# ElusAegis/metal-msm-gpu-acceleration

Hardware: AMD Instinct MI355X
Metric: BN254 G1 MSM/s at log_size=20 (5 instances) (higher is better)
Workload: dtype u32x8 (256-bit Montgomery integer)

## Files before the change

### include/msm_amd.h

```cpp
#ifndef MSM_AMD_H
#define MSM_AMD_H

#include <stddef.h>
#include <stdint.h>

#ifdef __cplusplus
extern "C" {
#endif

typedef struct msm_amd_ctx msm_amd_ctx;

enum {
  MSM_AMD_OK = 0,
  MSM_AMD_DEVICE_NOT_FOUND = 1,
  MSM_AMD_LIBRARY_ERROR = 2,
  MSM_AMD_FUNCTION_ERROR = 3,
  MSM_AMD_PIPELINE_ERROR = 4,
  MSM_AMD_INPUT_ERROR = 5,
  MSM_AMD_FILE_OPEN_ERROR = 6,
  MSM_AMD_DESERIALIZATION_ERROR = 7,
  MSM_AMD_INVALID_DATA = 8
};

enum {
// ... 235 lines not shown
  MSM_AMD_RAW_FE_SQR_WIDE = 33,
  MSM_AMD_RAW_FE_MUL2_WIDE = 34
};
int msm_amd_test_op_raw(msm_amd_ctx* ctx, int op, const uint32_t* a, const uint32_t* b, uint32_t* out, size_t count);
int msm_amd_test_op_raw_host(int op, const uint32_t* a, const uint32_t* b, uint32_t* out, size_t count);

int msm_amd_test_hold(msm_amd_ctx* ctx, uint32_t max_ms, void** handle);
int msm_amd_test_release(msm_amd_ctx* ctx, void* handle);

enum {
  MSM_AMD_TP_C = 0, MSM_AMD_TP_W, MSM_AMD_TP_W_DIGITS, MSM_AMD_TP_N, MSM_AMD_TP_N_SCALARS, MSM_AMD_TP_LB, MSM_AMD_TP_NB,
  MSM_AMD_TP_CH, MSM_AMD_TP_HB, MSM_AMD_TP_MB, MSM_AMD_TP_FB, MSM_AMD_TP_Q, MSM_AMD_TP_TILED, MSM_AMD_TP_BALLOT,
  MSM_AMD_TP_WIDE_DIGITS, MSM_AMD_TP_LONE,
  MSM_AMD_TP_TOTAL_ITEMS, MSM_AMD_TP_MULTI_COUNT, MSM_AMD_TP_DEFERRED,
  MSM_AMD_TP_RED_GROUP, MSM_AMD_TP_RB_THREADS, MSM_AMD_TP_INSTANCES, MSM_AMD_TP_WORKSPACE, MSM_AMD_TP_FRONT_THREADS,
  MSM_AMD_TEST_PLAN_WORDS
};
int msm_amd_test_last_plan(msm_amd_ctx* ctx, uint32_t j, uint32_t* out, size_t count);
enum {
  MSM_AMD_STAGE_DIGITS = 0,
  MSM_AMD_STAGE_SORTED = 1,
  MSM_AMD_STAGE_BUCKET_SIZE = 2,
  MSM_AMD_STAGE_BUCKET_START = 3,
  MSM_AMD_STAGE_ITEM_START = 4,
  MSM_AMD_STAGE_WIN_ITEMS = 5,
  MSM_AMD_STAGE_ORDER = 6,
  MSM_AMD_STAGE_MULTI_LIST = 7,
  MSM_AMD_STAGE_BUCKETS = 8,
  MSM_AMD_STAGE_PARTIAL = 9
};
// ... 63 lines not shown
```

### metal-msm-gpu-acceleration_amd/__init__.py

```python
from __future__ import annotations

import ctypes
import os
from ctypes import POINTER, c_char_p, c_float, c_int, c_size_t, c_uint32, c_uint64, c_void_p

_HERE = os.path.dirname(os.path.abspath(__file__))
LIB_PATH = os.environ.get("MSM_AMD_LIB") or os.path.join(_HERE, "libmsm_amd.so")

(OK, DEVICE_NOT_FOUND, LIBRARY_ERROR, FUNCTION_ERROR, PIPELINE_ERROR, INPUT_ERROR, FILE_OPEN_ERROR,
 DESERIALIZATION_ERROR, INVALID_DATA) = range(9)
SCALAR_MONT_LE, SCALAR_CANON_LE, SCALAR_CANON_BE32 = 0, 1, 2
POINT_H2C_AFFINE, POINT_ARK_PROJECTIVE, POINT_ARK_AFFINE, POINT_JAC_BE32, POINT_PREPARED, POINT_TABLES = 0, 1, 2, 3, 4, 5
POINT_BYTES = {POINT_H2C_AFFINE: 64, POINT_ARK_PROJECTIVE: 96, POINT_ARK_AFFINE: 72, POINT_JAC_BE32: 96}
(OP_UINT_ADD, OP_UINT_SUB, OP_UINT_PROD, OP_UINT_SHL, OP_UINT_SHR, OP_FP_ADD, OP_FP_SUB, OP_FP_MUL, OP_FP_NEG,
 OP_FP_POW, OP_EC_ADD, OP_EC_MUL, OP_EC_MADD, OP_EC_DBL, OP_FP29_MUL, OP_FP29_SQR, OP_FP29_SUB_K4E30,
 OP_FP29_SUB_K8E30, OP_FP29_SUB_K8E31, OP_FP29_SUB_K16E30, OP_FP29_SUB_K16E31, OP_FP29_ROUNDTRIP, OP_EC29_MADD,
 OP_EC29_ADD, OP_EC29_MADD_CHAIN, OP_EC29_ADD_CHAIN, OP_EC29_MMADD, OP_H64_FP_MUL, OP_H64_FP_ADD, OP_H64_FP_SUB,
 OP_H64_EC_ADD, OP_H64_EC_DBL, OP_FP29_MUL_KARATSUBA, OP_FP29_LOCKSTEP_PAIR, OP_FP29_LOCKSTEP_MIX,
 OP_FP29_LOCKSTEP_TRIPLE, OP_FP29_MUL2_KARATSUBA, OP_H64_FP_INV, OP_H64_FP_INV_FERMAT) = range(39)
(RAW_FE_MUL, RAW_FE_SQR, RAW_FE_MUL2, RAW_FE_SUB_K4E30, RAW_FE_SUB_K8E30, RAW_FE_SUB_K8E31, RAW_FE_SUB_K16E30,
 RAW_FE_SUB_K16E31, RAW_FE_NORM, RAW_FE_NEG, RAW_FE_NEG_WIDE, RAW_FE_CANONICAL, RAW_FE_TO_EXT, RAW_FE_PACK_UNPACK,
 RAW_FE_ZERO, RAW_PT_MADD, RAW_PT_MMADD, RAW_PT_ADD_NZ, RAW_PT_ADD, RAW_PT_DOUBLE) = range(20)
RAW_FE_MUL_WIDE, RAW_FE_SQR_WIDE, RAW_FE_MUL2_WIDE = range(32, 35)
RAW_IN_WORDS, RAW_OUT_WORDS = 36, 40
# ... 32 lines not shown
    "msm_amd_set_bases_cache_verify",
    "msm_amd_scalar_bytes", "msm_amd_point_bytes", "msm_amd_shard_owner",
    "msm_amd_shard_count", "msm_amd_ctx_device", "msm_amd_pin_thread_to_device", "msm_amd_gather_init",
    "msm_amd_gather_size", "msm_amd_gather_all", "msm_amd_gather_last_error", "msm_amd_gather_destroy",
    "msm_amd_host_msm", "msm_amd_tuned_split", "msm_amd_host_threads", "msm_amd_generate_instance_host", "msm_amd_test_op_ifma",
    "msm_amd_test_last_plan", "msm_amd_test_stage_copy", "msm_amd_test_fill_workspaces",
    "msm_amd_g2_point_bytes", "msm_amd_msm_g2", "msm_amd_msm_g2_device", "msm_amd_host_msm_g2",
    "msm_amd_test_g2_progression", "msm_amd_test_op_g2", "msm_amd_test_op_g2_host",
    "msm_amd_g2_bases_upload", "msm_amd_g2_bases_prepare_device", "msm_amd_msm_g2_prepared",
    "msm_amd_g2_tables_build", "msm_amd_g2_tables_build_device", "msm_amd_g2_tables_info", "msm_amd_g2_tables_free",
    "msm_amd_msm_g2_tables", "msm_amd_test_g2_tables_read", "msm_amd_test_g2_table_host",
]

TEST_PLAN_FIELDS = ("c", "W", "W_digits", "n", "n_scalars", "lb", "nb", "CH", "hb", "mb", "fb", "Q", "tiled", "ballot",
                    "wide_digits", "lone", "total_items", "multi_count", "deferred", "red_group", "rb_threads",
                    "instances", "workspace", "front_threads")
(STAGE_DIGITS, STAGE_SORTED, STAGE_BUCKET_SIZE, STAGE_BUCKET_START, STAGE_ITEM_START, STAGE_WIN_ITEMS, STAGE_ORDER,
 STAGE_MULTI_LIST, STAGE_BUCKETS, STAGE_PARTIAL) = range(10)


AFTER_SORT_FN = ctypes.CFUNCTYPE(None, c_void_p)


class Timings(ctypes.Structure):
    _fields_ = [("convert_ms", c_float), ("digits_ms", c_float), ("sort_ms", c_float), ("accumulate_ms", c_float),
                ("reduce_ms", c_float), ("final_ms", c_float), ("total_gpu_ms", c_float), ("n", c_uint32),
                ("window_size", c_uint32), ("num_windows", c_uint32), ("reserved", c_uint32),
                ("accumulate_kernel_ms", c_float), ("reserved2", c_float * 3)]


class MsmError(RuntimeError):
# ... 741 lines not shown
```

### metal-msm-gpu-acceleration_amd/csrc/k_sort.hip

```cpp
#include <algorithm>

#include "device_common.hip.h"
#include "launch.h"

namespace msm_amd {

constexpr int kSortThreads = 1024;

template <typename D, int C = 0>
__global__ void __launch_bounds__(256)
digits_kernel(const u256* __restrict__ scalars, uint32_t n, uint32_t c_arg, uint32_t W_arg, int scalars_mont,
              D* __restrict__ digits) {
  constexpr uint32_t kSignShift = 8 * sizeof(D) - 1;
  const uint32_t c = C > 0 ? (uint32_t)C : c_arg;
  const uint32_t W = C > 0 ? (uint32_t)(254 / (C > 0 ? C : 1) + 1) : W_arg;
  __builtin_amdgcn_s_setprio(kFrontPriority);
  const uint32_t t = blockIdx.x * blockDim.x + threadIdx.x;
  if (t >= n) return;
  u256 k = load_u256(&scalars[t]);
  if (scalars_mont) {
    k = Fr::from_mont(k);
  } else {
#pragma unroll 1
    for (int i = 0; i < 5; ++i) k = Fr::reduce_once(k);
  }
  const uint32_t half = 1u << (c - 1);
  uint32_t carry = 0;
#pragma unroll
  for (uint32_t w = 0; w < W; ++w) {
    const uint32_t start = w * c;
    uint32_t v = (start < 256 ? u256_extract_bits(k, start, c) : 0u) + carry;
    uint32_t neg = 0;
    carry = 0;
    if (v > half) {
      v = (1u << c) - v;
      neg = 1;
      carry = 1;
    }
    digits[(size_t)w * n + t] = (D)(v | (neg << kSignShift));
  }
}

constexpr uint32_t kFineCap = 28672;

template <typename D>
__global__ void __launch_bounds__(kSortThreads)
coarse_hist_kernel(const D* __restrict__ digits, uint32_t n, uint32_t fb, uint32_t nhi, uint32_t chunk,
                   uint32_t* __restrict__ coarse_cnt ) {
  constexpr uint32_t kMagMask = (1u << (8 * sizeof(D) - 1)) - 1u;
  __builtin_amdgcn_s_setprio(kFrontPriority);
  extern __shared__ uint32_t lds_u32[];
  const uint32_t q = blockIdx.x, Q = gridDim.x, w = blockIdx.y;
  for (uint32_t i = threadIdx.x; i < nhi; i += blockDim.x) lds_u32[i] = 0;
  __syncthreads();
// ... 48 lines not shown
    hi &= ~((uint32_t)(bal >> 32) ^ (uint32_t)s);
  }
  const uint32_t rank = __builtin_amdgcn_mbcnt_hi(hi, __builtin_amdgcn_mbcnt_lo(lo, 0u));
  const uint32_t count = __popc(lo) + __popc(hi);
  const uint32_t leader = lo ? (uint32_t)__builtin_ctz(lo) : 32u + (uint32_t)__builtin_ctz(hi | 0x80000000u);
  uint32_t base = 0;
  if (valid && rank == 0) base = atomicAdd(&cursors[key], count);
  base = (uint32_t)__builtin_amdgcn_ds_bpermute((int)(leader << 2), (int)base);
  return base + rank;
}

template <typename D, bool BALLOT>
__global__ void __launch_bounds__(kSortThreads)
coarse_scatter_kernel(const D* __restrict__ digits, uint32_t n, uint32_t hb, uint32_t fb, uint32_t chunk,
                      const uint32_t* __restrict__ coarse_base , uint32_t* __restrict__ tmp_idx,
                      uint16_t* __restrict__ tmp_fine) {
  __builtin_amdgcn_s_setprio(kFrontPriority);
  extern __shared__ uint32_t lds_u32[];
  const uint32_t nhi = 1u << hb;
  const uint32_t q = blockIdx.x, Q = gridDim.x, w = blockIdx.y;
  const uint32_t* base = coarse_base + ((size_t)w * Q + q) * nhi;
  for (uint32_t i = threadIdx.x; i < nhi; i += blockDim.x) lds_u32[i] = base[i];
  __syncthreads();
  const uint32_t lo = q * chunk;
  const uint32_t hi_end = min(n, lo + chunk);
  constexpr uint32_t kSignShift = 8 * sizeof(D) - 1;
  constexpr uint32_t kMagMask = (1u << kSignShift) - 1u;
  const D* dw = digits + (size_t)w * n;
  uint32_t* ti = tmp_idx + (size_t)w * n;
  uint16_t* tf = tmp_fine + (size_t)w * n;
  const uint32_t fmask = (1u << fb) - 1u;
  if (BALLOT) {
    for (uint32_t t0 = lo; t0 < hi_end; t0 += blockDim.x) {
      const uint32_t t = t0 + threadIdx.x;
      const uint32_t v = t < hi_end ? (uint32_t)dw[t] : 0u;
      const uint32_t m = v & kMagMask;
      const uint32_t slot = m - 1;
      const uint32_t pos = wave_claim(m ? slot >> fb : 0u, hb, m != 0, lds_u32);
      if (m) {
        ti[pos] = t | ((v >> kSignShift) << 31);
        tf[pos] = (uint16_t)(slot & fmask);
      }
    }
    return;
  }
  for (uint32_t t = lo + threadIdx.x; t < hi_end; t += blockDim.x) {
    const uint32_t v = dw[t];
    const uint32_t m = v & kMagMask;
    if (m) {
      const uint32_t slot = m - 1;
      const uint32_t pos = atomicAdd(&lds_u32[slot >> fb], 1u);
      ti[pos] = t | ((v >> kSignShift) << 31);
      tf[pos] = (uint16_t)(slot & fmask);
    }
  }
}


__global__ void __launch_bounds__(kSortThreads)
mid_hist_kernel(const uint16_t* __restrict__ tmp_fine, uint32_t n, uint32_t nhi, uint32_t fb, uint32_t nmid,
                const uint32_t* __restrict__ region_start, uint32_t* __restrict__ mid_cnt ) {
  __builtin_amdgcn_s_setprio(kFrontPriority);
  extern __shared__ uint32_t lds_u32[];
  const uint32_t q = blockIdx.x, Q2 = gridDim.x, R = blockIdx.y, w = R / nhi, r = R % nhi;
  for (uint32_t i = threadIdx.x; i < nmid; i += blockDim.x) lds_u32[i] = 0;
  __syncthreads();
  const uint32_t rs = region_start[(size_t)w * (nhi + 1) + r], re = region_start[(size_t)w * (nhi + 1) + r + 1];
  const uint32_t chunk = (((re - rs) + Q2 - 1) / Q2 + 63u) & ~63u;
// ... 123 lines not shown
#pragma unroll
    for (uint32_t e = 0; e < kTilePerThread; ++e) {
      if (reg[e] != 0xFFFFFFFFu) {
        const uint32_t p = off[reg[e]] + rank[e];
        st_idx[p] = pay[e];
        st_fine[p] = (uint16_t)fin[e];
        st_reg[p] = (uint8_t)reg[e];
      }
    }
    __syncthreads();
    const uint32_t tile_total = scratch[32];
    for (uint32_t j = threadIdx.x; j < tile_total; j += blockDim.x) {
      const uint32_t r = st_reg[j];
      const uint32_t gp = gbase[r] + (j - off[r]);
      out_idx[gp] = st_idx[j];
      out_fine[gp] = st_fine[j];
    }
    __syncthreads();
  }
}

template <typename D>
__global__ void __launch_bounds__(kSortThreads)
coarse_scatter_tiled_kernel(const D* __restrict__ digits, uint32_t n, uint32_t hb, uint32_t fb, uint32_t chunk,
                            const uint32_t* __restrict__ coarse_base, uint32_t* __restrict__ tmp_idx,
                            uint16_t* __restrict__ tmp_fine) {
  __builtin_amdgcn_s_setprio(kFrontPriority);
  extern __shared__ uint32_t lds_u32[];
  constexpr uint32_t kSignShift = 8 * sizeof(D) - 1;
  constexpr uint32_t kMagMask = (1u << kSignShift) - 1u;
  const uint32_t nhi = 1u << hb;
  const uint32_t q = blockIdx.x, Q = gridDim.x, w = blockIdx.y;
  const uint32_t lo = q * chunk, hi = min(n, lo + chunk);
  const D* dw = digits + (size_t)w * n;
  const uint32_t fmask = (1u << fb) - 1u;
  auto load = [&](uint32_t t, uint32_t* pay, uint32_t* fin, uint32_t* reg) {
    const uint32_t v = dw[t];
    const uint32_t m = v & kMagMask;
    if (!m) return false;
    const uint32_t slot = m - 1;
    *pay = t | ((v >> kSignShift) << 31);
    *fin = slot & fmask;
    *reg = slot >> fb;
    return true;
  };
  tile_scatter(lo, hi, nhi, hb, load, coarse_base + ((size_t)w * Q + q) * nhi, tmp_idx + (size_t)w * n,
               tmp_fine + (size_t)w * n, lds_u32);
}

__global__ void __launch_bounds__(kSortThreads)
mid_scatter_tiled_kernel(const uint32_t* __restrict__ tmp_idx, const uint16_t* __restrict__ tmp_fine, uint32_t n,
                         uint32_t nhi, uint32_t fb, uint32_t mb, const uint32_t* __restrict__ region_start,
                         const uint32_t* __restrict__ mid_base, uint32_t* __restrict__ tmp_idx2,
                         uint16_t* __restrict__ tmp_fine2) {
  __builtin_amdgcn_s_setprio(kFrontPriority);
  extern __shared__ uint32_t lds_u32[];
  const uint32_t nmid = 1u << mb;
  const uint32_t q = blockIdx.x, Q2 = gridDim.x, R = blockIdx.y, w = R / nhi, r = R % nhi;
  const uint32_t rs = region_start[(size_t)w * (nhi + 1) + r], re = region_start[(size_t)w * (nhi + 1) + r + 1];
  const uint32_t chunk = (((re - rs) + Q2 - 1) / Q2 + 63u) & ~63u;
  const uint32_t lo = min(re, rs + q * chunk), hi = min(re, lo + chunk);
  const uint32_t* ti = tmp_idx + (size_t)w * n;
  const uint16_t* tf = tmp_fine + (size_t)w * n;
  const uint32_t fmask = (1u << fb) - 1u;
  auto load = [&](uint32_t t, uint32_t* pay, uint32_t* fin, uint32_t* reg) {
    const uint32_t f = tf[t];
    *pay = ti[t];
    *fin = f & fmask;
    *reg = f >> fb;
    return true;
  };
  tile_scatter(lo, hi, nmid, mb, load, mid_base + ((size_t)R * Q2 + q) * nmid, tmp_idx2 + (size_t)w * n,
               tmp_fine2 + (size_t)w * n, lds_u32);
}

template <bool BALLOT>
__global__ void __launch_bounds__(kSortThreads)
fine_sort_kernel(const uint32_t* __restrict__ tmp_idx, const uint16_t* __restrict__ tmp_fine, uint32_t n,
                 uint32_t lb, uint32_t fb, const uint32_t* __restrict__ region_start,
                 uint32_t* __restrict__ sorted, uint32_t* __restrict__ bucket_size) {
  __builtin_amdgcn_s_setprio(kFrontPriority);
  extern __shared__ uint32_t lds_u32[];
  const uint32_t nfine = 1u << fb;
  const uint32_t nhi = gridDim.x;
  const uint32_t hi = blockIdx.x, w = blockIdx.y;
  uint32_t* bins = lds_u32;
  uint32_t* scratch = lds_u32 + nfine;
  uint32_t* staging = lds_u32 + nfine + 32;
  const uint32_t rs = region_start[(size_t)w * (nhi + 1) + hi];
  const uint32_t re = region_start[(size_t)w * (nhi + 1) + hi + 1];
  const uint32_t size = re - rs;
  const uint32_t* ti = tmp_idx + (size_t)w * n + rs;
  const uint16_t* tf = tmp_fine + (size_t)w * n + rs;
  uint32_t* out = sorted + (size_t)w * n + rs;
  for (uint32_t i = threadIdx.x; i < nfine; i += blockDim.x) bins[i] = 0;
  __syncthreads();
#pragma unroll 1
  for (uint32_t i = threadIdx.x; i < size; i += blockDim.x) atomicAdd(&bins[tf[i]], 1u);
  __syncthreads();
  const uint32_t cnt = (threadIdx.x < nfine) ? bins[threadIdx.x] : 0u;
  uint32_t total;
  const uint32_t start = block_exclusive_scan(cnt, scratch, &total);
  if (threadIdx.x < nfine) {
    bins[threadIdx.x] = start;
    const uint32_t slot = (hi << fb) | threadIdx.x;
    if (slot < (1u << lb)) bucket_size[((size_t)w << lb) + slot] = cnt;
  }
  __syncthreads();
  if (size <= kFineCap) {
    if (BALLOT) {
#pragma unroll 1
      for (uint32_t i0 = 0; i0 < size; i0 += blockDim.x) {
        const uint32_t i = i0 + threadIdx.x;
        const bool valid = i < size;
        const uint32_t pos = wave_claim(valid ? (uint32_t)tf[i] : 0u, fb, valid, bins);
        if (valid) staging[pos] = ti[i];
      }
    } else {
#pragma unroll 1
      for (uint32_t i = threadIdx.x; i < size; i += blockDim.x) {
        const uint32_t pos = atomicAdd(&bins[tf[i]], 1u);
        staging[pos] = ti[i];
      }
    }
    __syncthreads();
  #pragma unroll 1
  for (uint32_t i = threadIdx.x; i < size; i += blockDim.x) out[i] = staging[i];
  } else {
  #pragma unroll 1
  for (uint32_t i = threadIdx.x; i < size; i += blockDim.x) {
      const uint32_t pos = atomicAdd(&bins[tf[i]], 1u);
      out[pos] = ti[i];
    }
  }
}

__device__ __forceinline__ uint32_t window_scan_lds(uint32_t* tot, uint32_t* scratch, uint32_t nb) {
  const uint32_t per = (nb + blockDim.x - 1) / blockDim.x;
  const uint32_t first = threadIdx.x * per;
  uint32_t local = 0;
#pragma unroll 1
  for (uint32_t j = 0; j < per; ++j) {
    const uint32_t d = first + j;
    if (d < nb) local += tot[d + (d >> 5)];
  }
  uint32_t total;
  uint32_t run = block_exclusive_scan(local, scratch, &total);
// ... 209 lines not shown
  const size_t tile = std::min<size_t>((size_t)1 << lb, kPlanTile);
  return (tile + (tile >> 5) + 33) * 4;
}

int sort_set_attributes(const char** failed) {
  const int max_lds = 160 * 1024;
  struct { const void* fn; const char* name; } ks[] = {
      {(const void*)plan_kernel, "plan_kernel"},
      {(const void*)coarse_scatter_kernel<uint16_t, false>, "coarse_scatter_kernel<u16>"},
      {(const void*)coarse_scatter_kernel<uint32_t, false>, "coarse_scatter_kernel<u32>"},
      {(const void*)coarse_scatter_kernel<uint16_t, true>, "coarse_scatter_kernel<u16, ballot>"},
      {(const void*)coarse_scatter_kernel<uint32_t, true>, "coarse_scatter_kernel<u32, ballot>"},
      {(const void*)coarse_scatter_tiled_kernel<uint16_t>, "coarse_scatter_tiled_kernel<u16>"},
      {(const void*)coarse_scatter_tiled_kernel<uint32_t>, "coarse_scatter_tiled_kernel<u32>"},
      {(const void*)mid_scatter_tiled_kernel, "mid_scatter_tiled_kernel"},
      {(const void*)fine_sort_kernel<false>, "fine_sort_kernel"},
      {(const void*)fine_sort_kernel<true>, "fine_sort_kernel<ballot>"}};
  for (auto& k : ks) {
    if (hipFuncSetAttribute(k.fn, hipFuncAttributeMaxDynamicSharedMemorySize, max_lds) != hipSuccess) {
      (void)hipGetLastError();
      *failed = k.name;
      return 1;
    }
  }
  return 0;
}

void launch_digits(hipStream_t st, const Plan& p, const u256* scalars, int scalars_mont, void* digits) {
  const dim3 grid((p.n_scalars + 255) / 256), block(256);
#define LAUNCH_DIGITS_C(D, CC)                                                                                      \
  hipLaunchKernelGGL((digits_kernel<D, CC>), grid, block, 0, st, scalars, p.n_scalars, p.c, p.W_digits, scalars_mont, \
                     (D*)digits)
  if (p.W_digits == 254 / p.c + 1) {
    if (p.wide_digits && p.c == 17) { LAUNCH_DIGITS_C(uint32_t, 17); return; }
    if (p.wide_digits && p.c == 16) { LAUNCH_DIGITS_C(uint32_t, 16); return; }
    if (!p.wide_digits && p.c == 15) { LAUNCH_DIGITS_C(uint16_t, 15); return; }
    if (!p.wide_digits && p.c == 13) { LAUNCH_DIGITS_C(uint16_t, 13); return; }
  }
#undef LAUNCH_DIGITS_C
  if (p.wide_digits)
    hipLaunchKernelGGL(digits_kernel<uint32_t>, grid, block, 0, st, scalars, p.n_scalars, p.c, p.W_digits, scalars_mont,
                       (uint32_t*)digits);
  else
    hipLaunchKernelGGL(digits_kernel<uint16_t>, grid, block, 0, st, scalars, p.n_scalars, p.c, p.W_digits, scalars_mont,
                       (uint16_t*)digits);
}

void launch_sort(hipStream_t st, const Plan& p, const SortBuffers& b) {
  const uint32_t nhi = 1u << p.hb, nmid = 1u << p.mb, nfine = 1u << p.fb;
  const uint32_t fb1 = p.mb + p.fb;
  if (p.wide_digits)
    hipLaunchKernelGGL(coarse_hist_kernel<uint32_t>, dim3(p.Q, p.W), dim3(p.front_threads), nhi * 4, st,
                       (const uint32_t*)b.digits, p.n, fb1, nhi, p.chunk, b.coarse_cnt);
  else
    hipLaunchKernelGGL(coarse_hist_kernel<uint16_t>, dim3(p.Q, p.W), dim3(p.front_threads), nhi * 4, st,
                       (const uint16_t*)b.digits, p.n, fb1, nhi, p.chunk, b.coarse_cnt);
  hipLaunchKernelGGL(coarse_prefix_kernel, dim3(p.W), dim3(1024), 0, st, b.coarse_cnt, p.Q, nhi, b.region_start);
  const bool bc = (p.ballot & 1u) != 0, bf = (p.ballot & 2u) != 0;
#define LAUNCH_COARSE_SCATTER(D, B)                                                                                 \
  hipLaunchKernelGGL((coarse_scatter_kernel<D, B>), dim3(p.Q, p.W), dim3(p.front_threads), nhi * 4, st,             \
                     (const D*)b.digits, p.n, p.hb, fb1, p.chunk, (const uint32_t*)b.coarse_cnt, b.tmp_idx, b.tmp_fine)
  const bool tiled = p.tiled && p.front_threads == kSortThreads && nhi <= kTileMaxRegions && nmid <= kTileMaxRegions;
  if (tiled) {
    if (p.wide_digits)
      hipLaunchKernelGGL(coarse_scatter_tiled_kernel<uint32_t>, dim3(p.Q, p.W), dim3(p.tile_threads), kTileLdsBytes, st,
                         (const uint32_t*)b.digits, p.n, p.hb, fb1, p.chunk, (const uint32_t*)b.coarse_cnt, b.tmp_idx,
                         b.tmp_fine);
    else
      hipLaunchKernelGGL(coarse_scatter_tiled_kernel<uint16_t>, dim3(p.Q, p.W), dim3(p.tile_threads), kTileLdsBytes, st,
                         (const uint16_t*)b.digits, p.n, p.hb, fb1, p.chunk, (const uint32_t*)b.coarse_cnt, b.tmp_idx,
                         b.tmp_fine);
  } else if (p.wide_digits) {
    if (bc) LAUNCH_COARSE_SCATTER(uint32_t, true); else LAUNCH_COARSE_SCATTER(uint32_t, false);
  } else {
    if (bc) LAUNCH_COARSE_SCATTER(uint16_t, true); else LAUNCH_COARSE_SCATTER(uint16_t, false);
  }
#undef LAUNCH_COARSE_SCATTER
  const uint32_t* fine_idx = b.tmp_idx;
  const uint16_t* fine_fine = b.tmp_fine;
  const uint32_t* fine_regions = b.region_start;
  uint32_t fine_nhi = nhi;
  if (p.mb) {
    hipLaunchKernelGGL(mid_hist_kernel, dim3(p.Q2, nhi * p.W), dim3(p.front_threads), nmid * 4, st,
                       (const uint16_t*)b.tmp_fine, p.n, nhi, p.fb, nmid, (const uint32_t*)b.region_start, b.mid_cnt);
    hipLaunchKernelGGL(mid_prefix_kernel, dim3(nhi * p.W), dim3(1024), 0, st, b.mid_cnt, p.Q2, nhi, nmid,
                       (const uint32_t*)b.region_start, b.region_start2);
// ... 2 lines not shown
                         (const uint32_t*)b.tmp_idx, (const uint16_t*)b.tmp_fine, p.n, nhi, p.fb, p.mb,
                         (const uint32_t*)b.region_start, (const uint32_t*)b.mid_cnt, b.tmp_idx2, b.tmp_fine2);
    else if (bc)
      hipLaunchKernelGGL(mid_scatter_kernel<true>, dim3(p.Q2, nhi * p.W), dim3(p.front_threads), nmid * 4, st,
                         (const uint32_t*)b.tmp_idx, (const uint16_t*)b.tmp_fine, p.n, nhi, p.fb, nmid,
                         (const uint32_t*)b.region_start, (const uint32_t*)b.mid_cnt, b.tmp_idx2, b.tmp_fine2);
    else
      hipLaunchKernelGGL(mid_scatter_kernel<false>, dim3(p.Q2, nhi * p.W), dim3(p.front_threads), nmid * 4, st,
                         (const uint32_t*)b.tmp_idx, (const uint16_t*)b.tmp_fine, p.n, nhi, p.fb, nmid,
                         (const uint32_t*)b.region_start, (const uint32_t*)b.mid_cnt, b.tmp_idx2, b.tmp_fine2);
    fine_idx = b.tmp_idx2;
    fine_fine = b.tmp_fine2;
    fine_regions = b.region_start2;
    fine_nhi = nhi * nmid;
  }
  if (bf)
    hipLaunchKernelGGL(fine_sort_kernel<true>, dim3(fine_nhi, p.W), dim3(std::max(p.front_threads, nfine)),
                       (kFineCap + nfine + 32) * 4, st, fine_idx, fine_fine, p.n, p.lb, p.fb, fine_regions, b.sorted,
                       b.bucket_size);
  else
    hipLaunchKernelGGL(fine_sort_kernel<false>, dim3(fine_nhi, p.W), dim3(std::max(p.front_threads, nfine)),
                       (kFineCap + nfine + 32) * 4, st, fine_idx, fine_fine, p.n, p.lb, p.fb, fine_regions, b.sorted,
                       b.bucket_size);
  const unsigned tiles = (unsigned)((p.nb + kPlanTile - 1) / kPlanTile);
  if (tiles > 1)
    hipLaunchKernelGGL(plan_tile_sums_kernel, dim3(tiles, p.W), dim3(p.front_threads), 0, st,
                       (const uint32_t*)b.bucket_size, p.lb, p.CH, b.tile_sums);
  hipLaunchKernelGGL(plan_kernel, dim3(tiles, p.W), dim3(p.front_threads), lds_plan_bytes(p.lb), st,
                     (const uint32_t*)b.bucket_size, p.lb, p.CH, (const uint2*)b.tile_sums, b.bucket_start,
                     b.item_start, b.win_items);
  const unsigned size_threads = p.front_threads;
  const unsigned gb = (unsigned)((p.total_buckets + size_threads * kSizeChunks - 1) / (size_threads * kSizeChunks));
  hipLaunchKernelGGL(size_hist_kernel, dim3(gb), dim3(size_threads), (p.CH + 1) * 4, st,
                     (const uint32_t*)b.bucket_size, (uint32_t)p.total_buckets, p.CH, b.size_bins);
  hipLaunchKernelGGL(size_scan_kernel, dim3(1), dim3(1024), 0, st, b.size_bins, (p.CH + 1) * gb, b.win_items, p.W,
                     b.counters);
  hipLaunchKernelGGL(size_scatter_kernel, dim3(gb), dim3(size_threads), (2 * (p.CH + 1) + 2) * 4, st,
                     (const uint32_t*)b.bucket_size, (uint32_t)p.total_buckets, p.CH, (const uint32_t*)b.size_bins, b.order,
// ... 13 lines not shown
```

### metal-msm-gpu-acceleration_amd/csrc/launch.h

```cpp
#pragma once
#include <hip/hip_runtime.h>
#include <stddef.h>
#include <stdint.h>

#include "bn254_ec29.hip.h"

namespace msm_amd {

constexpr int kSegLog = 3;

struct Plan {
  uint32_t n, c, W;
  uint32_t n_scalars, W_digits;
  bool wide_digits;
  uint32_t lb, nb;
  uint32_t Q, chunk;
  uint32_t hb, mb, fb;
  uint32_t Q2;
  uint32_t tile_threads;
  uint32_t tiled;
  uint32_t ballot;
  uint32_t front_threads;
  uint32_t CH;
  uint32_t red_L, red_H;
  uint32_t rb_threads;
  uint32_t red_group;
  size_t total_buckets, total_segs, partial_count, max_items;
};

struct PlanCounters {
  uint32_t total_items;
  uint32_t multi_count;
  uint32_t pad[2];
};

struct SortBuffers {
  void* digits;
// ... 9 lines not shown
  uint32_t* bucket_start;
  uint32_t* item_start;
  uint32_t* win_items;
  uint2* tile_sums;
  uint32_t* size_bins;
  uint32_t* sorted;
  uint2* order;
  uint32_t* multi_list;
  uint32_t* redo_list;
  PlanCounters* counters;
};

int sort_set_attributes(const char** failed);
void launch_build_tables(hipStream_t st, const Affine* in, uint32_t n, uint32_t c, uint32_t W, AffPacked* tables);
void launch_digits(hipStream_t st, const Plan& p, const u256* scalars, int scalars_mont, void* digits);
void launch_sort(hipStream_t st, const Plan& p, const SortBuffers& b);
void launch_be32_to_le(hipStream_t st, const uint32_t* in, size_t words, uint32_t* out);
void launch_ark_affine_to_affine(hipStream_t st, const uint8_t* in, uint32_t n, Affine* out);

void launch_accumulate(hipStream_t st, const Plan& p, const void* bases, int wide, const SortBuffers& b, PtI* buckets,
                       PtI* partials, int variant, uint32_t lds_bytes, hipEvent_t before_kernel, hipEvent_t after_kernel);

void launch_combine(hipStream_t st, const Plan& p, const SortBuffers& b, PtI* buckets, PtI* partials);

int reduce_set_attributes(const char** failed);
constexpr uint32_t kReduceGroup = 16;
constexpr uint32_t kReduceGroupMin = 4;
constexpr size_t kReduceResidentLanes = 160 * 1024;
size_t reduce_scratch_elems(uint32_t lb);
void launch_reduce(hipStream_t st, const Plan& p, const PtI* buckets, const uint32_t* bucket_size, PtI* S, PtI* T,
                   Jacobian* partial);
// ... 29 lines not shown
```

### metal-msm-gpu-acceleration_amd/csrc/msm_host.hip

```cpp
#include <hip/hip_runtime.h>

#include <algorithm>
#include <atomic>
#include <chrono>
#include <cmath>
#include <cstdio>
#include <cstdlib>
#include <cstring>
#include <condition_variable>
#include <mutex>
#include <string>
#include <thread>
#include <vector>

#include "../../include/msm_amd.h"
#include "device_common.hip.h"
#include "launch.h"
#include "launch_g2.h"
#include "host_fq64.h"
#include "test_ops.hip.h"
#include "test_ops_g2.hip.h"

using namespace msm_amd;

// ... 397 lines not shown
    if (p.mb || p.hb + extra > 7) p.mb += extra; else p.hb += extra;
  }
  while (p.mb + p.fb > 16) {
    ++p.hb;
    --p.mb;
  }
  p.tiled = (p.mb != 0 && windows == 0) ? 1u : 0u;
  if (const char* e = std::getenv("MSM_AMD_TILED")) p.tiled = std::atoi(e) != 0;
  p.tile_threads = 1024;
  if (const char* e = std::getenv("MSM_AMD_TILE_THREADS")) {
    const int v = std::atoi(e);
    if (v == 256 || v == 512 || v == 1024) p.tile_threads = (uint32_t)v;
  }
  p.ballot = kDefaultBallot;
  if (const char* e = std::getenv("MSM_AMD_BALLOT")) p.ballot = (uint32_t)std::atoi(e) & 3u;
  p.Q2 = 1;
  if (p.mb) {
    const uint32_t regions = p.W << p.hb;
    p.Q2 = std::max(1u, 1024u / regions);
    while (p.Q2 > 1 && (n >> p.hb) / p.Q2 < 4096) p.Q2 >>= 1;
  }
  const double mean_len = (double)n / (double)p.nb;
  uint32_t ch = 16;
  while (ch < 512 && (double)ch < mean_len + 5.0 * std::sqrt(mean_len)) ch <<= 1;
  while (ch > 16 && (size_t)p.W * p.nb + ((size_t)p.W * n) / ch < 262144) ch >>= 1;
  if (const char* e = std::getenv("MSM_AMD_CH")) {
    const int v = std::atoi(e);
    if (v >= 16 && v <= 512 && (v & (v - 1)) == 0) ch = (uint32_t)v;
  }
  p.CH = ch;
// ... 286 lines not shown
  const u256* sc = nullptr;
  const Affine* pts = nullptr;
  int sc_mont = 0;
  if ((rc = convert_inputs(ctx, w, fs, scalar_layout, tb ? MSM_AMD_POINT_PREPARED : point_layout, d_scalars, d_points,
                           p.n_scalars, &sc, &sc_mont, &pts)))
    return rc;
  const AffPacked* bases = tb ? (const AffPacked*)tb->d_tables
                              : (prepared ? (const AffPacked*)d_points
                                          : (fill ? (const AffPacked*)fill : (const AffPacked*)w.bases29.p));
#if defined(MSM_AMD_EXPERIMENTS)
  if (wide) launch_convert_bases_wide(fs, pts, p.n, (AffWide*)w.bases29.p);
#endif
  if (!prepared && !wide)
    launch_convert_bases(fs, pts, p.n, fill ? fill : (AffPacked*)w.bases29.p);
  HIP_TRY(ctx, hipEventRecord(slot.ev[EV_CONVERT], fs));
  launch_digits(fs, p, sc, sc_mont, sb.digits);
  HIP_TRY(ctx, hipEventRecord(slot.ev[EV_DIGITS], fs));
  launch_sort(fs, p, sb);
  HIP_TRY(ctx, hipEventRecord(slot.ev[EV_SORT], fs));
  if (fs != st) {
    HIP_TRY(ctx, hipEventRecord(w.front_done, fs));
    HIP_TRY(ctx, hipStreamWaitEvent(st, w.front_done, 0));
  }
  if (w.reduce_pending) {
    if (rs != st) HIP_TRY(ctx, hipStreamWaitEvent(st, w.reduce_done, 0));
    w.reduce_pending = false;
  }
  launch_accumulate(st, p, bases, wide ? 1 : 0, sb, (PtI*)w.buckets.p, (PtI*)w.item_partials.p,
                    ctx->acc_variant, ctx->acc_lds, slot.ev[EV_ACC_K0], slot.ev[EV_ACC_K1]);
  HIP_TRY(ctx, hipEventRecord(w.acc_done, st));
  w.acc_pending = true;

  if (rs != st) HIP_TRY(ctx, hipStreamWaitEvent(rs, w.acc_done, 0));
// ... 1921 lines not shown
  v[MSM_AMD_TP_MB] = p.mb;
  v[MSM_AMD_TP_FB] = p.fb;
  v[MSM_AMD_TP_Q] = p.Q;
  v[MSM_AMD_TP_TILED] = p.tiled;
  v[MSM_AMD_TP_BALLOT] = p.ballot;
  v[MSM_AMD_TP_WIDE_DIGITS] = p.wide_digits ? 1u : 0u;
  v[MSM_AMD_TP_LONE] = B->lone ? 1u : 0u;
  v[MSM_AMD_TP_TOTAL_ITEMS] = pc.total_items;
  v[MSM_AMD_TP_MULTI_COUNT] = pc.multi_count;
  v[MSM_AMD_TP_DEFERRED] = pc.pad[0];
  v[MSM_AMD_TP_RED_GROUP] = p.red_group;
  v[MSM_AMD_TP_RB_THREADS] = p.rb_threads;
  v[MSM_AMD_TP_INSTANCES] = (uint32_t)B->n_inst;
  v[MSM_AMD_TP_WORKSPACE] = (uint32_t)B->ws_index[j];
  v[MSM_AMD_TP_FRONT_THREADS] = p.front_threads;
  std::memcpy(out, v, sizeof v);
  return MSM_AMD_OK;
}

int msm_amd_test_stage_copy(msm_amd_ctx* ctx, uint32_t j, int which, void* out, size_t* bytes) {
  if (!ctx || !bytes) return fail(ctx, MSM_AMD_INPUT_ERROR, "bad test_stage_copy arguments");
  std::lock_guard<std::mutex> g(ctx->mu);
  const Batch* B = nullptr;
  if (int rc = tap_batch(ctx, j, &B)) return rc;
  const Plan& p = B->plans[j];
  Workspace& w = ctx->ws[B->ws_index[j]];
  PlanCounters pc;
  std::memcpy(&pc, B->slots[j].h_partial + B->slots[j].h_partial_cap, sizeof pc);
  const DeviceBuf* src = nullptr;
  size_t dev_bytes = 0, out_bytes = 0;
// ... 171 lines not shown
  sb.counters = (PlanCounters*)w.counters.p;

  HIP_TRY(ctx, hipEventRecord(g.ev[G2State::EV_G2_START], st));
  const u256* sc = nullptr;
  const Affine* unused = nullptr;
  int sc_mont = 0;
  if ((rc = convert_inputs(ctx, w, st, scalar_layout, MSM_AMD_POINT_PREPARED, d_scalars, nullptr, p.n_scalars, &sc,
                           &sc_mont, &unused)))
    return rc;
  const Aff2Packed* bases = tb ? (const Aff2Packed*)tb->d_tables
                               : (prepared ? (const Aff2Packed*)d_points : (const Aff2Packed*)g.bases.p);
  if (!prepared)
    launch_convert_bases_g2(st, d_points, g2_point_layout == MSM_AMD_G2_POINT_ARK_AFFINE, (uint32_t)n,
                            (Aff2Packed*)g.bases.p);
  HIP_TRY(ctx, hipEventRecord(g.ev[G2State::EV_G2_CONVERT], st));
  launch_digits(st, p, sc, sc_mont, sb.digits);
  HIP_TRY(ctx, hipEventRecord(g.ev[G2State::EV_G2_DIGITS], st));
  launch_sort(st, p, sb);
  HIP_TRY(ctx, hipEventRecord(g.ev[G2State::EV_G2_SORT], st));
  launch_accumulate_g2(st, p, bases, sb, (PtI2*)g.buckets.p, (PtI2*)g.item_partials.p);
  launch_combine_g2(st, p, sb, (PtI2*)g.buckets.p, (PtI2*)g.item_partials.p);
  HIP_TRY(ctx, hipEventRecord(g.ev[G2State::EV_G2_ACC], st));
  launch_reduce_g2(st, p, (const PtI2*)g.buckets.p, (const uint32_t*)w.bsize.p, (PtI2*)g.S.p, (PtI2*)g.T.p,
                   (Jacobian2*)g.partial.p);
  HIP_TRY(ctx, hipGetLastError());
  HIP_TRY(ctx, hipMemcpyAsync(g.h_partial, g.partial.p, p.partial_count * sizeof(Jacobian2), hipMemcpyDeviceToHost, st));
  HIP_TRY(ctx, hipEventRecord(g.ev[G2State::EV_G2_REDUCE], st));
  const hipError_t we = wait_event(g.ev[G2State::EV_G2_REDUCE], ctx->wait_timeout_ms);
  if (we == hipErrorNotReady) {
    ctx->stalled = true;
    return fail(ctx, MSM_AMD_PIPELINE_ERROR,
                "timed out after " + std::to_string(ctx->wait_timeout_ms) + " ms waiting for the G2 MSM");
  }
// ... 293 lines not shown
```

Baseline: 789.7.

## Fuse digit extraction with coarse histogram and pack fine bits into sort index

Result: faster. 808.1 (median of 6 runs) (+2.3%).

```diff
diff --git a/include/msm_amd.h b/include/msm_amd.h
--- a/include/msm_amd.h
+++ b/include/msm_amd.h
@@ -273,6 +273,8 @@
   MSM_AMD_TP_WIDE_DIGITS, MSM_AMD_TP_LONE,
   MSM_AMD_TP_TOTAL_ITEMS, MSM_AMD_TP_MULTI_COUNT, MSM_AMD_TP_DEFERRED,
   MSM_AMD_TP_RED_GROUP, MSM_AMD_TP_RB_THREADS, MSM_AMD_TP_INSTANCES, MSM_AMD_TP_WORKSPACE, MSM_AMD_TP_FRONT_THREADS,
+  MSM_AMD_TP_FUSED_FRONT,
+  MSM_AMD_TP_PACKED,
   MSM_AMD_TEST_PLAN_WORDS
 };
 int msm_amd_test_last_plan(msm_amd_ctx* ctx, uint32_t j, uint32_t* out, size_t count);
diff --git a/metal-msm-gpu-acceleration_amd/__init__.py b/metal-msm-gpu-acceleration_amd/__init__.py
--- a/metal-msm-gpu-acceleration_amd/__init__.py
+++ b/metal-msm-gpu-acceleration_amd/__init__.py
@@ -70,7 +70,7 @@
 
 TEST_PLAN_FIELDS = ("c", "W", "W_digits", "n", "n_scalars", "lb", "nb", "CH", "hb", "mb", "fb", "Q", "tiled", "ballot",
                     "wide_digits", "lone", "total_items", "multi_count", "deferred", "red_group", "rb_threads",
-                    "instances", "workspace", "front_threads")
+                    "instances", "workspace", "front_threads", "fused_front", "packed")
 (STAGE_DIGITS, STAGE_SORTED, STAGE_BUCKET_SIZE, STAGE_BUCKET_START, STAGE_ITEM_START, STAGE_WIN_ITEMS, STAGE_ORDER,
  STAGE_MULTI_LIST, STAGE_BUCKETS, STAGE_PARTIAL) = range(10)
 
diff --git a/metal-msm-gpu-acceleration_amd/csrc/k_sort.hip b/metal-msm-gpu-acceleration_amd/csrc/k_sort.hip
--- a/metal-msm-gpu-acceleration_amd/csrc/k_sort.hip
+++ b/metal-msm-gpu-acceleration_amd/csrc/k_sort.hip
@@ -7,17 +7,10 @@
 
 constexpr int kSortThreads = 1024;
 
-template <typename D, int C = 0>
-__global__ void __launch_bounds__(256)
-digits_kernel(const u256* __restrict__ scalars, uint32_t n, uint32_t c_arg, uint32_t W_arg, int scalars_mont,
-              D* __restrict__ digits) {
-  constexpr uint32_t kSignShift = 8 * sizeof(D) - 1;
+template <int C, typename Emit>
+__device__ __forceinline__ void scalar_digits(u256 k, int scalars_mont, uint32_t c_arg, uint32_t W_arg, Emit emit) {
   const uint32_t c = C > 0 ? (uint32_t)C : c_arg;
   const uint32_t W = C > 0 ? (uint32_t)(254 / (C > 0 ? C : 1) + 1) : W_arg;
-  __builtin_amdgcn_s_setprio(kFrontPriority);
-  const uint32_t t = blockIdx.x * blockDim.x + threadIdx.x;
-  if (t >= n) return;
-  u256 k = load_u256(&scalars[t]);
   if (scalars_mont) {
     k = Fr::from_mont(k);
   } else {
@@ -26,7 +19,8 @@
   }
   const uint32_t half = 1u << (c - 1);
   uint32_t carry = 0;
-#pragma unroll
+  constexpr int kUnroll = C > 0 ? 254 / (C > 0 ? C : 1) + 1 : 1;
+#pragma unroll kUnroll
   for (uint32_t w = 0; w < W; ++w) {
     const uint32_t start = w * c;
     uint32_t v = (start < 256 ? u256_extract_bits(k, start, c) : 0u) + carry;
@@ -37,7 +31,52 @@
       neg = 1;
       carry = 1;
     }
+    emit(w, v, neg);
+  }
+}
+
+template <typename D, int C = 0>
+__global__ void __launch_bounds__(256)
+digits_kernel(const u256* __restrict__ scalars, uint32_t n, uint32_t c_arg, uint32_t W_arg, int scalars_mont,
+              D* __restrict__ digits) {
+  constexpr uint32_t kSignShift = 8 * sizeof(D) - 1;
+  __builtin_amdgcn_s_setprio(kFrontPriority);
+  const uint32_t t = blockIdx.x * blockDim.x + threadIdx.x;
+  if (t >= n) return;
+  scalar_digits<C>(load_u256(&scalars[t]), scalars_mont, c_arg, W_arg, [&](uint32_t w, uint32_t v, uint32_t neg) {
     digits[(size_t)w * n + t] = (D)(v | (neg << kSignShift));
+  });
+}
+
+constexpr uint32_t kDigitsThreads = 256;
+constexpr uint32_t kDigitsSpan = kDigitsThreads * 8;
+template <typename D, int C = 0>
+__global__ void __launch_bounds__(kDigitsThreads)
+digits_hist_kernel(const u256* __restrict__ scalars, uint32_t n, uint32_t c_arg, uint32_t W_arg, int scalars_mont,
+                   uint32_t fb, uint32_t nhi, uint32_t chunk, D* __restrict__ digits,
+                   uint32_t* __restrict__ coarse_cnt ) {
+  constexpr uint32_t kSignShift = 8 * sizeof(D) - 1;
+  const uint32_t W = C > 0 ? (uint32_t)(254 / (C > 0 ? C : 1) + 1) : W_arg;
+  __builtin_amdgcn_s_setprio(kFrontPriority);
+  extern __shared__ uint32_t lds_u32[];
+  const uint32_t q = blockIdx.y, Q = gridDim.y;
+  const uint32_t lo = q * chunk + blockIdx.x * kDigitsSpan;
+  const uint32_t hi = min(min(n, (q + 1) * chunk), lo + kDigitsSpan);
+  if (lo >= hi) return;
+  for (uint32_t i = threadIdx.x; i < W * nhi; i += blockDim.x) lds_u32[i] = 0;
+  __syncthreads();
+#pragma unroll 1
+  for (uint32_t t = lo + threadIdx.x; t < hi; t += blockDim.x) {
+    scalar_digits<C>(load_u256(&scalars[t]), scalars_mont, c_arg, W_arg, [&](uint32_t w, uint32_t v, uint32_t neg) {
+      digits[(size_t)w * n + t] = (D)(v | (neg << kSignShift));
+      if (v) atomicAdd(&lds_u32[w * nhi + ((v - 1) >> fb)], 1u);
+    });
+  }
+  __syncthreads();
+  for (uint32_t i = threadIdx.x; i < W * nhi; i += blockDim.x) {
+    const uint32_t w = i / nhi, r = i - w * nhi;
+    const uint32_t cnt = lds_u32[i];
+    if (cnt) atomicAdd(&coarse_cnt[((size_t)w * Q + q) * nhi + r], cnt);
   }
 }
 
@@ -116,7 +155,7 @@
 __global__ void __launch_bounds__(kSortThreads)
 coarse_scatter_kernel(const D* __restrict__ digits, uint32_t n, uint32_t hb, uint32_t fb, uint32_t chunk,
                       const uint32_t* __restrict__ coarse_base , uint32_t* __restrict__ tmp_idx,
-                      uint16_t* __restrict__ tmp_fine) {
+                      uint16_t* __restrict__ tmp_fine, uint32_t packed) {
   __builtin_amdgcn_s_setprio(kFrontPriority);
   extern __shared__ uint32_t lds_u32[];
   const uint32_t nhi = 1u << hb;
@@ -140,8 +179,12 @@
       const uint32_t slot = m - 1;
       const uint32_t pos = wave_claim(m ? slot >> fb : 0u, hb, m != 0, lds_u32);
       if (m) {
-        ti[pos] = t | ((v >> kSignShift) << 31);
-        tf[pos] = (uint16_t)(slot & fmask);
+        if (packed) {
+          ti[pos] = (slot & fmask) | (t << fb) | ((v >> kSignShift) << 31);
+        } else {
+          ti[pos] = t | ((v >> kSignShift) << 31);
+          tf[pos] = (uint16_t)(slot & fmask);
+        }
       }
     }
     return;
@@ -152,8 +195,12 @@
     if (m) {
       const uint32_t slot = m - 1;
       const uint32_t pos = atomicAdd(&lds_u32[slot >> fb], 1u);
-      ti[pos] = t | ((v >> kSignShift) << 31);
-      tf[pos] = (uint16_t)(slot & fmask);
+      if (packed) {
+        ti[pos] = (slot & fmask) | (t << fb) | ((v >> kSignShift) << 31);
+      } else {
+        ti[pos] = t | ((v >> kSignShift) << 31);
+        tf[pos] = (uint16_t)(slot & fmask);
+      }
     }
   }
 }
@@ -307,7 +354,7 @@
       const uint32_t r = st_reg[j];
       const uint32_t gp = gbase[r] + (j - off[r]);
       out_idx[gp] = st_idx[j];
-      out_fine[gp] = st_fine[j];
+      if (out_fine) out_fine[gp] = st_fine[j];
     }
     __syncthreads();
   }
@@ -317,7 +364,7 @@
 __global__ void __launch_bounds__(kSortThreads)
 coarse_scatter_tiled_kernel(const D* __restrict__ digits, uint32_t n, uint32_t hb, uint32_t fb, uint32_t chunk,
                             const uint32_t* __restrict__ coarse_base, uint32_t* __restrict__ tmp_idx,
-                            uint16_t* __restrict__ tmp_fine) {
+                            uint16_t* __restrict__ tmp_fine, uint32_t packed) {
   __builtin_amdgcn_s_setprio(kFrontPriority);
   extern __shared__ uint32_t lds_u32[];
   constexpr uint32_t kSignShift = 8 * sizeof(D) - 1;
@@ -333,12 +380,13 @@
     if (!m) return false;
     const uint32_t slot = m - 1;
     *pay = t | ((v >> kSignShift) << 31);
+    if (packed) *pay = (slot & fmask) | (t << fb) | ((v >> kSignShift) << 31);
     *fin = slot & fmask;
     *reg = slot >> fb;
     return true;
   };
   tile_scatter(lo, hi, nhi, hb, load, coarse_base + ((size_t)w * Q + q) * nhi, tmp_idx + (size_t)w * n,
-               tmp_fine + (size_t)w * n, lds_u32);
+               packed ? nullptr : tmp_fine + (size_t)w * n, lds_u32);
 }
 
 __global__ void __launch_bounds__(kSortThreads)
@@ -367,7 +415,7 @@
                tmp_fine2 + (size_t)w * n, lds_u32);
 }
 
-template <bool BALLOT>
+template <bool BALLOT, bool PACKED>
 __global__ void __launch_bounds__(kSortThreads)
 fine_sort_kernel(const uint32_t* __restrict__ tmp_idx, const uint16_t* __restrict__ tmp_fine, uint32_t n,
                  uint32_t lb, uint32_t fb, const uint32_t* __restrict__ region_start,
@@ -386,10 +434,13 @@
   const uint32_t* ti = tmp_idx + (size_t)w * n + rs;
   const uint16_t* tf = tmp_fine + (size_t)w * n + rs;
   uint32_t* out = sorted + (size_t)w * n + rs;
+  const uint32_t fmask = nfine - 1u;
+  auto fine_of = [&](uint32_t i) { return PACKED ? (ti[i] & fmask) : (uint32_t)tf[i]; };
+  auto unpack = [&](uint32_t v) { return PACKED ? ((v & 0x80000000u) | ((v & 0x7FFFFFFFu) >> fb)) : v; };
   for (uint32_t i = threadIdx.x; i < nfine; i += blockDim.x) bins[i] = 0;
   __syncthreads();
 #pragma unroll 1
-  for (uint32_t i = threadIdx.x; i < size; i += blockDim.x) atomicAdd(&bins[tf[i]], 1u);
+  for (uint32_t i = threadIdx.x; i < size; i += blockDim.x) atomicAdd(&bins[fine_of(i)], 1u);
   __syncthreads();
   const uint32_t cnt = (threadIdx.x < nfine) ? bins[threadIdx.x] : 0u;
   uint32_t total;
@@ -406,24 +457,28 @@
       for (uint32_t i0 = 0; i0 < size; i0 += blockDim.x) {
         const uint32_t i = i0 + threadIdx.x;
         const bool valid = i < size;
-        const uint32_t pos = wave_claim(valid ? (uint32_t)tf[i] : 0u, fb, valid, bins);
-        if (valid) staging[pos] = ti[i];
+        const uint32_t v = (PACKED && valid) ? ti[i] : 0u;
+        const uint32_t f = PACKED ? (v & fmask) : (valid ? (uint32_t)tf[i] : 0u);
+        const uint32_t pos = wave_claim(f, fb, valid, bins);
+        if (valid) staging[pos] = PACKED ? unpack(v) : ti[i];
       }
     } else {
 #pragma unroll 1
       for (uint32_t i = threadIdx.x; i < size; i += blockDim.x) {
-        const uint32_t pos = atomicAdd(&bins[tf[i]], 1u);
-        staging[pos] = ti[i];
+        const uint32_t v = ti[i];
+        const uint32_t pos = atomicAdd(&bins[PACKED ? (v & fmask) : (uint32_t)tf[i]], 1u);
+        staging[pos] = unpack(v);
       }
     }
     __syncthreads();
-  #pragma unroll 1
-  for (uint32_t i = threadIdx.x; i < size; i += blockDim.x) out[i] = staging[i];
+#pragma unroll 1
+    for (uint32_t i = threadIdx.x; i < size; i += blockDim.x) out[i] = staging[i];
   } else {
-  #pragma unroll 1
-  for (uint32_t i = threadIdx.x; i < size; i += blockDim.x) {
-      const uint32_t pos = atomicAdd(&bins[tf[i]], 1u);
-      out[pos] = ti[i];
+#pragma unroll 1
+    for (uint32_t i = threadIdx.x; i < size; i += blockDim.x) {
+      const uint32_t v = ti[i];
+      const uint32_t pos = atomicAdd(&bins[PACKED ? (v & fmask) : (uint32_t)tf[i]], 1u);
+      out[pos] = unpack(v);
     }
   }
 }
@@ -663,8 +718,10 @@
       {(const void*)coarse_scatter_tiled_kernel<uint16_t>, "coarse_scatter_tiled_kernel<u16>"},
       {(const void*)coarse_scatter_tiled_kernel<uint32_t>, "coarse_scatter_tiled_kernel<u32>"},
       {(const void*)mid_scatter_tiled_kernel, "mid_scatter_tiled_kernel"},
-      {(const void*)fine_sort_kernel<false>, "fine_sort_kernel"},
-      {(const void*)fine_sort_kernel<true>, "fine_sort_kernel<ballot>"}};
+      {(const void*)fine_sort_kernel<false, false>, "fine_sort_kernel"},
+      {(const void*)fine_sort_kernel<true, false>, "fine_sort_kernel<ballot>"},
+      {(const void*)fine_sort_kernel<false, true>, "fine_sort_kernel<packed>"},
+      {(const void*)fine_sort_kernel<true, true>, "fine_sort_kernel<ballot, packed>"}};
   for (auto& k : ks) {
     if (hipFuncSetAttribute(k.fn, hipFuncAttributeMaxDynamicSharedMemorySize, max_lds) != hipSuccess) {
       (void)hipGetLastError();
@@ -695,10 +752,31 @@
                        (uint16_t*)digits);
 }
 
-void launch_sort(hipStream_t st, const Plan& p, const SortBuffers& b) {
+void launch_digits_hist(hipStream_t st, const Plan& p, const u256* scalars, int scalars_mont, const SortBuffers& b) {
+  const uint32_t nhi = 1u << p.hb;
+  const uint32_t fb1 = p.mb + p.fb;
+  const dim3 grid((p.chunk + kDigitsSpan - 1) / kDigitsSpan, p.Q), block(kDigitsThreads);
+  const size_t lds = (size_t)p.W * nhi * 4;
+  (void)hipMemsetAsync(b.coarse_cnt, 0, (size_t)p.W * p.Q * nhi * sizeof(uint32_t), st);
+#define LAUNCH_DIGITS_HIST_C(D, CC)                                                                                 \
+  hipLaunchKernelGGL((digits_hist_kernel<D, CC>), grid, block, lds, st, scalars, p.n_scalars, p.c, p.W_digits,       \
+                     scalars_mont, fb1, nhi, p.chunk, (D*)b.digits, b.coarse_cnt)
+  if (p.W_digits == 254 / p.c + 1) {
+    if (p.wide_digits && p.c == 17) { LAUNCH_DIGITS_HIST_C(uint32_t, 17); return; }
+    if (p.wide_digits && p.c == 16) { LAUNCH_DIGITS_HIST_C(uint32_t, 16); return; }
+    if (!p.wide_digits && p.c == 15) { LAUNCH_DIGITS_HIST_C(uint16_t, 15); return; }
+    if (!p.wide_digits && p.c == 13) { LAUNCH_DIGITS_HIST_C(uint16_t, 13); return; }
+  }
+  if (p.wide_digits) LAUNCH_DIGITS_HIST_C(uint32_t, 0); else LAUNCH_DIGITS_HIST_C(uint16_t, 0);
+#undef LAUNCH_DIGITS_HIST_C
+}
+
+void launch_sort(hipStream_t st, const Plan& p, const SortBuffers& b, bool have_hist) {
   const uint32_t nhi = 1u << p.hb, nmid = 1u << p.mb, nfine = 1u << p.fb;
   const uint32_t fb1 = p.mb + p.fb;
-  if (p.wide_digits)
+  const uint32_t packed = p.packed ? 1u : 0u;
+  if (have_hist) {
+  } else if (p.wide_digits)
     hipLaunchKernelGGL(coarse_hist_kernel<uint32_t>, dim3(p.Q, p.W), dim3(p.front_threads), nhi * 4, st,
                        (const uint32_t*)b.digits, p.n, fb1, nhi, p.chunk, b.coarse_cnt);
   else
@@ -707,18 +785,19 @@
   hipLaunchKernelGGL(coarse_prefix_kernel, dim3(p.W), dim3(1024), 0, st, b.coarse_cnt, p.Q, nhi, b.region_start);
   const bool bc = (p.ballot & 1u) != 0, bf = (p.ballot & 2u) != 0;
 #define LAUNCH_COARSE_SCATTER(D, B)                                                                                 \
-  hipLaunchKernelGGL((coarse_scatter_kernel<D, B>), dim3(p.Q, p.W), dim3(p.front_threads), nhi * 4, st,             \
-                     (const D*)b.digits, p.n, p.hb, fb1, p.chunk, (const uint32_t*)b.coarse_cnt, b.tmp_idx, b.tmp_fine)
+  hipLaunchKernelGGL((coarse_scatter_kernel<D, B>), dim3(p.Q, p.W), dim3(p.front_threads), nhi * 4, st,              \
+                     (const D*)b.digits, p.n, p.hb, fb1, p.chunk, (const uint32_t*)b.coarse_cnt, b.tmp_idx, b.tmp_fine, \
+                     packed)
   const bool tiled = p.tiled && p.front_threads == kSortThreads && nhi <= kTileMaxRegions && nmid <= kTileMaxRegions;
   if (tiled) {
     if (p.wide_digits)
       hipLaunchKernelGGL(coarse_scatter_tiled_kernel<uint32_t>, dim3(p.Q, p.W), dim3(p.tile_threads), kTileLdsBytes, st,
                          (const uint32_t*)b.digits, p.n, p.hb, fb1, p.chunk, (const uint32_t*)b.coarse_cnt, b.tmp_idx,
-                         b.tmp_fine);
+                         b.tmp_fine, packed);
     else
       hipLaunchKernelGGL(coarse_scatter_tiled_kernel<uint16_t>, dim3(p.Q, p.W), dim3(p.tile_threads), kTileLdsBytes, st,
                          (const uint16_t*)b.digits, p.n, p.hb, fb1, p.chunk, (const uint32_t*)b.coarse_cnt, b.tmp_idx,
-                         b.tmp_fine);
+                         b.tmp_fine, packed);
   } else if (p.wide_digits) {
     if (bc) LAUNCH_COARSE_SCATTER(uint32_t, true); else LAUNCH_COARSE_SCATTER(uint32_t, false);
   } else {
@@ -751,14 +830,16 @@
     fine_regions = b.region_start2;
     fine_nhi = nhi * nmid;
   }
-  if (bf)
-    hipLaunchKernelGGL(fine_sort_kernel<true>, dim3(fine_nhi, p.W), dim3(std::max(p.front_threads, nfine)),
-                       (kFineCap + nfine + 32) * 4, st, fine_idx, fine_fine, p.n, p.lb, p.fb, fine_regions, b.sorted,
-                       b.bucket_size);
-  else
-    hipLaunchKernelGGL(fine_sort_kernel<false>, dim3(fine_nhi, p.W), dim3(std::max(p.front_threads, nfine)),
-                       (kFineCap + nfine + 32) * 4, st, fine_idx, fine_fine, p.n, p.lb, p.fb, fine_regions, b.sorted,
-                       b.bucket_size);
+#define LAUNCH_FINE_SORT(B, PK)                                                                                     \
+  hipLaunchKernelGGL((fine_sort_kernel<B, PK>), dim3(fine_nhi, p.W), dim3(std::max(p.front_threads, nfine)),         \
+                     (kFineCap + nfine + 32) * 4, st, fine_idx, fine_fine, p.n, p.lb, p.fb, fine_regions, b.sorted,  \
+                     b.bucket_size)
+  if (packed) {
+    if (bf) LAUNCH_FINE_SORT(true, true); else LAUNCH_FINE_SORT(false, true);
+  } else {
+    if (bf) LAUNCH_FINE_SORT(true, false); else LAUNCH_FINE_SORT(false, false);
+  }
+#undef LAUNCH_FINE_SORT
   const unsigned tiles = (unsigned)((p.nb + kPlanTile - 1) / kPlanTile);
   if (tiles > 1)
     hipLaunchKernelGGL(plan_tile_sums_kernel, dim3(tiles, p.W), dim3(p.front_threads), 0, st,
diff --git a/metal-msm-gpu-acceleration_amd/csrc/launch.h b/metal-msm-gpu-acceleration_amd/csrc/launch.h
--- a/metal-msm-gpu-acceleration_amd/csrc/launch.h
+++ b/metal-msm-gpu-acceleration_amd/csrc/launch.h
@@ -21,6 +21,8 @@
   uint32_t tiled;
   uint32_t ballot;
   uint32_t front_threads;
+  bool fused_front;
+  bool packed;
   uint32_t CH;
   uint32_t red_L, red_H;
   uint32_t rb_threads;
@@ -60,7 +62,8 @@
 int sort_set_attributes(const char** failed);
 void launch_build_tables(hipStream_t st, const Affine* in, uint32_t n, uint32_t c, uint32_t W, AffPacked* tables);
 void launch_digits(hipStream_t st, const Plan& p, const u256* scalars, int scalars_mont, void* digits);
-void launch_sort(hipStream_t st, const Plan& p, const SortBuffers& b);
+void launch_digits_hist(hipStream_t st, const Plan& p, const u256* scalars, int scalars_mont, const SortBuffers& b);
+void launch_sort(hipStream_t st, const Plan& p, const SortBuffers& b, bool have_hist = false);
 void launch_be32_to_le(hipStream_t st, const uint32_t* in, size_t words, uint32_t* out);
 void launch_ark_affine_to_affine(hipStream_t st, const uint8_t* in, uint32_t n, Affine* out);
 
diff --git a/metal-msm-gpu-acceleration_amd/csrc/msm_host.hip b/metal-msm-gpu-acceleration_amd/csrc/msm_host.hip
--- a/metal-msm-gpu-acceleration_amd/csrc/msm_host.hip
+++ b/metal-msm-gpu-acceleration_amd/csrc/msm_host.hip
@@ -435,6 +435,8 @@
   }
   p.ballot = kDefaultBallot;
   if (const char* e = std::getenv("MSM_AMD_BALLOT")) p.ballot = (uint32_t)std::atoi(e) & 3u;
+  p.fused_front = windows == 0;
+  p.packed = p.mb == 0 && n >= 1 && floor_log2(std::max<size_t>(n - 1, 1)) + 1 + 1 + p.fb <= 32;
   p.Q2 = 1;
   if (p.mb) {
     const uint32_t regions = p.W << p.hb;
@@ -751,9 +753,9 @@
   if (!prepared && !wide)
     launch_convert_bases(fs, pts, p.n, fill ? fill : (AffPacked*)w.bases29.p);
   HIP_TRY(ctx, hipEventRecord(slot.ev[EV_CONVERT], fs));
-  launch_digits(fs, p, sc, sc_mont, sb.digits);
+  if (p.fused_front) launch_digits_hist(fs, p, sc, sc_mont, sb); else launch_digits(fs, p, sc, sc_mont, sb.digits);
   HIP_TRY(ctx, hipEventRecord(slot.ev[EV_DIGITS], fs));
-  launch_sort(fs, p, sb);
+  launch_sort(fs, p, sb, p.fused_front);
   HIP_TRY(ctx, hipEventRecord(slot.ev[EV_SORT], fs));
   if (fs != st) {
     HIP_TRY(ctx, hipEventRecord(w.front_done, fs));
@@ -2705,6 +2707,8 @@
   v[MSM_AMD_TP_INSTANCES] = (uint32_t)B->n_inst;
   v[MSM_AMD_TP_WORKSPACE] = (uint32_t)B->ws_index[j];
   v[MSM_AMD_TP_FRONT_THREADS] = p.front_threads;
+  v[MSM_AMD_TP_FUSED_FRONT] = p.fused_front ? 1u : 0u;
+  v[MSM_AMD_TP_PACKED] = p.packed ? 1u : 0u;
   std::memcpy(out, v, sizeof v);
   return MSM_AMD_OK;
 }
@@ -2906,9 +2910,9 @@
     launch_convert_bases_g2(st, d_points, g2_point_layout == MSM_AMD_G2_POINT_ARK_AFFINE, (uint32_t)n,
                             (Aff2Packed*)g.bases.p);
   HIP_TRY(ctx, hipEventRecord(g.ev[G2State::EV_G2_CONVERT], st));
-  launch_digits(st, p, sc, sc_mont, sb.digits);
+  if (p.fused_front) launch_digits_hist(st, p, sc, sc_mont, sb); else launch_digits(st, p, sc, sc_mont, sb.digits);
   HIP_TRY(ctx, hipEventRecord(g.ev[G2State::EV_G2_DIGITS], st));
-  launch_sort(st, p, sb);
+  launch_sort(st, p, sb, p.fused_front);
   HIP_TRY(ctx, hipEventRecord(g.ev[G2State::EV_G2_SORT], st));
   launch_accumulate_g2(st, p, bases, sb, (PtI2*)g.buckets.p, (PtI2*)g.item_partials.p);
   launch_combine_g2(st, p, sb, (PtI2*)g.buckets.p, (PtI2*)g.item_partials.p);
```
